# seemapoudel58/Physics_informed_image_segmentation

Hardware: AMD Instinct MI355X
Metric: training images/sec (512x512, Stage-II RD+PF loss) (higher is better)
Workload: dtype fp32 (fp16x3 split MFMA, power-of-two block scales; direct + Winograd convs); 1 GPU; C2: UNet(1,1,64) bs=8/GPU 512x512 Stage-II (lambda_RD=lambda_PF=1e-4, D=5, a=0.5, eps=0.05) AdamW lr=1e-5; global_batch=8, parallelism=dp1

## Files before the change

include/pis_capi.h:

```cpp
#ifndef PIS_CAPI_H
#define PIS_CAPI_H

#include <stddef.h>
#include <stdint.h>

#ifdef __cplusplus
extern "C" {
#endif

typedef void* pis_stream_t;

#define PIS_OK 0
#define PIS_ERR_ARG (-1)
#define PIS_ERR_LAUNCH (-2)
#define PIS_ERR_WORKSPACE (-3)

#define PIS_RELU 1
#define PIS_SCALE 2
#define PIS_MASK 4
#define PIS_ACCUMULATE 8
#define PIS_WINO_PREPARED 16
#define PIS_W_UNFLIPPED 32
#define PIS_FILTER_READY 64

// ... 27 lines not shown
#define PIS_TUNE_FUSED_STAGGER 25
#define PIS_TUNE_FUSED_WIDE 26
#define PIS_TUNE_FUSED_K128 27
#define PIS_TUNE_FUSED_PAIR 28
#define PIS_TUNE_DIRECT_H3 29
#define PIS_TUNE_DIRECT_WG 30
#define PIS_TUNE_WGRAD_T 31
#define PIS_TUNE_DIRECT_PIPE 32
#define PIS_TUNE_DIRECT_W8 33
#define PIS_TUNE_DIRECT_WSTRIP 34
#define PIS_TUNE_DIRECT_WBLOCKS 35
#define PIS_TUNE_HEAD_LOSS_ROWS 36
#define PIS_TUNE_DIRECT_WGRAD_ALL 37
#define PIS_TUNE_HEAD_LOSS_WIDE 38
#define PIS_TUNE_WGRAD_T_DEPTH 39
#define PIS_TUNE_DZ_VW 40
#define PIS_TUNE_GEMM_256 41
#define PIS_TUNE_LAST_WGRAD_MAIN 42
#define PIS_TUNE_DIRECT_W_VWALK 43
#define PIS_TUNE_DIRECT_WGRAD_MAIN 44
#define PIS_TUNE_GEMM_PRIO 45
#define PIS_TUNE_WINO_OUT_MPF 46
#define PIS_TUNE_WINO_F6 47
#define PIS_TUNE_WGRAD_OUT 48
#define PIS_TUNE_DIRECT_W_ROWS 49
#define PIS_TUNE_WINO_XFORM 50
#define PIS_TUNE_WINO_DGRAD_T 51
#define PIS_TUNE_PROB_VARIANT 52
#define PIS_TUNE_DIRECT_MFMA16 53
#define PIS_TUNE_EVOLVE_T 54
#define PIS_TUNE_EDT_PRUNE 55
#define PIS_TUNE_CONVT_WGRAD_TILE 56
#define PIS_TUNE_UNROLL_TB 57
#define PIS_TUNE_NKEYS 58
#define PIS_DEBUG_NOLOAD (1 << 16)
int pis_tune(int key, int value);
int pis_debug_gemm_nt(const float* A, const float* B, float* C, int M, int N, int K, int batch, int variant,
                      pis_stream_t stream);
int pis_debug_stream_probe(const float* a, const float* b, float* dst, int64_t n, float* partial, int grid,
                           pis_stream_t stream);

int pis_debug_band_probe(const float* a, int64_t n, int mode, float* partial, int grid, pis_stream_t stream);

int pis_arm_gemm_event(void* event);

int pis_stream_create(int priority, pis_stream_t* out);
int pis_stream_destroy(pis_stream_t stream);
int pis_stream_capture_status(pis_stream_t stream);

typedef void (*pis_launch_hook_t)(const char* kernel, int phase, pis_stream_t stream, double flop,
                                  void* user);
void pis_set_launch_hook(pis_launch_hook_t fn, void* user);

int pis_conv3x3_fwd(const float* x, int ldx, const float* w_krsc, const float* bias,
                    const float* scale, float* y, int ldy, int B, int H, int W, int Cin,
                    int Cout, int flags, pis_stream_t stream);
size_t pis_conv3x3_ex_ws(int B, int H, int W, int Cin, int Cout);
int pis_conv3x3_fwd_ex(const float* x, int ldx, const float* w_krsc, const float* bias,
                       const float* scale, float* y, int ldy, int B, int H, int W, int Cin, int Cout,
                       int flags, void* ws, size_t ws_bytes, pis_stream_t stream);
int pis_conv3x3_flip(const float* w_krsc, float* w_flip, int Cin, int Cout, pis_stream_t stream);
int pis_conv3x3_dgrad(const float* dz, int ldz, const float* w_flip, const float* mask, int ldm,
                      const float* scale, float* dx, int lddx, int B, int H, int W, int Cin,
                      int Cout, int flags, pis_stream_t stream);
int pis_conv3x3_dgrad_ex(const float* dz, int ldz, const float* w_flip, const float* mask, int ldm,
                         const float* scale, float* dx, int lddx, int B, int H, int W, int Cin,
                         int Cout, int flags, void* ws, size_t ws_bytes, pis_stream_t stream);
// ... 8 lines not shown
                           int B, int H, int W, int Cin, int Cout, int flags, void* ws, size_t ws_bytes,
                           const float* keep, pis_stream_t stream);
size_t pis_conv3x3_filter_bytes(int B, int H, int W, int Cin, int Cout, int dgrad);
int pis_conv3x3_filter(const float* w, int B, int H, int W, int Cin, int Cout, int dgrad, void* out,
                       size_t out_bytes, pis_stream_t stream);
typedef struct pis_filter_job {
  const float* w;
  void* out;
  size_t out_bytes;
  int B, H, W, Cin, Cout, dgrad;
} pis_filter_job;
#define PIS_FILTER_MAX_JOBS 40
int pis_conv3x3_filter_format(int B, int H, int W, int Cin, int Cout, int dgrad);
int pis_conv3x3_filters(const pis_filter_job* jobs, int n, pis_stream_t stream);
int pis_conv3x3_dgrad_direct(int B, int H, int W, int Cin, int Cout, int ldz, size_t ws_bytes);
int pis_conv3x3_bwd_prep(const float* dz, int ldz, int B, int H, int W, int Cin, int Cout, void* ws_dgrad,
                         size_t ws_dgrad_bytes, void* ws_wgrad, size_t ws_wgrad_bytes, pis_stream_t stream);
size_t pis_conv3x3_wgrad_ws(int B, int H, int W, int Cin, int Cout);
int pis_conv3x3_wgrad(const float* x, int ldx, const float* dz, int ldz, float* dw_krsc, float* db,
                      int B, int H, int W, int Cin, int Cout, int flags, void* ws, size_t ws_bytes,
                      pis_stream_t stream);

int pis_convt2x2_fwd(const float* x, int ldx, const float* w_ijoc, const float* bias, float* y,
                     int ldy, int B, int H, int W, int Cin, int Cout, pis_stream_t stream);
int pis_convt2x2_prep(const float* w_ijoc, float* w_cijo, int Cin, int Cout, pis_stream_t stream);
int pis_convt2x2_dgrad(const float* dy, int lddy, const float* w_cijo, const float* mask, int ldm,
                       float* dx, int lddx, int B, int H, int W, int Cin, int Cout, int flags,
                       pis_stream_t stream);
size_t pis_convt2x2_wgrad_ws(int B, int H, int W, int Cin, int Cout);
int pis_convt2x2_wgrad(const float* x, int ldx, const float* dy, int lddy, float* dw_ijoc,
                       float* db, int B, int H, int W, int Cin, int Cout, int flags, void* ws,
                       size_t ws_bytes, pis_stream_t stream);
int pis_debug_convt2x2_wgrad_tile_splits(int B, int H, int W, int Cin, int Cout);
int pis_debug_convt2x2_algo(int op, int B, int H, int W, int Cin, int Cout, int ld_src, int ld_dst, int aligned16);

int pis_maxpool2x2_fwd(const float* x, int ldx, float* y, int B, int H, int W, int C,
                       pis_stream_t stream);
int pis_maxpool2x2_bwd(const float* x, int ldx, const float* dy, const float* dskip, int ldskip,
                       float* dx, int lddx, int B, int H, int W, int C, pis_stream_t stream);

int pis_head_fwd(const float* x, int ldx, const float* w, const float* b, float* z, float* u,
                 int64_t npix, int C, pis_stream_t stream);
size_t pis_head_bwd_ws(int64_t npix, int C);
int pis_head_bwd(const float* x, int ldx, const float* w, const float* g, const float* u, float* dx,
                 int lddx, float* dw, float* db, int64_t npix, int C, int flags, void* ws,
                 size_t ws_bytes, pis_stream_t stream);

typedef struct pis_loss_params {
  float dice_w, bce_w;
  float rd_w, pf_w;
  float smooth;
  float D, a;
  float eps;
  float thr;
  int flags;
} pis_loss_params;
#define PIS_LOSS_ALL_TERMS 1
#define PIS_LOSS_CHAIN_SIGMOID 2
#define PIS_LOSS_NO_REACTION 4
#define PIS_LOSS_NTERMS 8
size_t pis_loss_ws(int B, int H, int W);
int pis_loss_fwd(const float* p, const float* t, int B, int H, int W, const pis_loss_params* prm,
                 float* out_terms, int* counts, float* scores, void* ws, size_t ws_bytes,
                 pis_stream_t stream);
int pis_loss_bwd(const float* p, const float* t, int B, int H, int W, const pis_loss_params* prm,
                 const float* terms, const float* grad_out, float* dst, int flags,
// ... 119 lines not shown
```

physics_informed_image_segmentation_amd/_hip.py:

```python
from __future__ import annotations

import ctypes
import os
from ctypes import c_double, c_float, c_int, c_int64, c_size_t, c_void_p
from typing import Optional

import torch

_HERE = os.path.dirname(os.path.abspath(__file__))
LIB_PATH = os.path.join(_HERE, "_lib", "libpis.so")

PIS_RELU, PIS_SCALE, PIS_MASK, PIS_ACCUMULATE, PIS_WINO_PREPARED, PIS_W_UNFLIPPED = 1, 2, 4, 8, 16, 32
PIS_FILTER_READY = 64
PIS_LOSS_ALL_TERMS, PIS_LOSS_CHAIN_SIGMOID, PIS_LOSS_NO_REACTION = 1, 2, 4
PIS_TUNE_LAST_WGRAD_MAIN = 42
PIS_TUNE_DIRECT_MFMA16 = 53
PIS_TUNE_PROB_VARIANT = 52
PIS_TUNE_EVOLVE_T = 54
PIS_TUNE_EDT_PRUNE = 55
PIS_TUNE_CONVT_WGRAD_TILE = 56
PIS_TUNE_UNROLL_TB = 57
PIS_UNROLL_MAX_STEPS = 1024
PIS_EVOLVE_CLAMP, PIS_EVOLVE_TILE_H, PIS_EVOLVE_TILE_W, PIS_EVOLVE_MAX_STEPS = 1, 32, 64, 65536
PIS_CACHE_IMG_U8, PIS_CACHE_IMG_F32, PIS_CACHE_MASK_BITS, PIS_CACHE_MASK_F32 = 0, 1, 0, 1
PIS_GRADNORM_SKIP_NONFINITE, PIS_GRADNORM_NSTATS = 1, 8
LOSS_NTERMS = 8
TERM_TOTAL, TERM_DICE, TERM_BCE, TERM_RD, TERM_PF, TERM_I, TERM_P, TERM_T = range(8)


class FilterJob(ctypes.Structure):
    _fields_ = [("w", c_void_p), ("out", c_void_p), ("out_bytes", c_size_t), ("B", c_int), ("H", c_int),
                ("W", c_int), ("Cin", c_int), ("Cout", c_int), ("dgrad", c_int)]


class LossParams(ctypes.Structure):
    _fields_ = [("dice_w", c_float), ("bce_w", c_float), ("rd_w", c_float), ("pf_w", c_float),
                ("smooth", c_float), ("D", c_float), ("a", c_float), ("eps", c_float),
                ("thr", c_float), ("flags", c_int)]


P, I, L, Z, Dbl = c_void_p, c_int, c_int64, c_size_t, c_double
LAUNCH_HOOK_T = ctypes.CFUNCTYPE(None, ctypes.c_char_p, c_int, c_void_p, ctypes.c_double, c_void_p)

_SIGNATURES = {
    "pis_set_launch_hook": ([LAUNCH_HOOK_T, P], None),
    "pis_arm_gemm_event": ([P], c_int),
    "pis_stream_create": ([I, ctypes.POINTER(c_void_p)], c_int),
    "pis_stream_destroy": ([P], c_int),
    "pis_stream_capture_status": ([P], c_int),
    "pis_version": ([], c_int),
    "pis_last_error": ([], ctypes.c_char_p),
    "pis_tune": ([I, I], c_int),
    "pis_debug_gemm_nt": ([P, P, P, I, I, I, I, I, P], c_int),
    "pis_debug_stream_probe": ([P, P, P, L, P, I, P], c_int),
    "pis_debug_band_probe": ([P, L, I, P, I, P], c_int),
    "pis_conv3x3_dgrad_direct": ([I, I, I, I, I, I, Z], c_int),
    "pis_conv3x3_bwd_prep": ([P, I, I, I, I, I, I, P, Z, P, Z, P], c_int),
    "pis_conv3x3_filter_bytes": ([I, I, I, I, I, I], c_size_t),
    "pis_conv3x3_filter_format": ([I, I, I, I, I, I], c_int),
    "pis_conv3x3_filter": ([P, I, I, I, I, I, I, P, Z, P], c_int),
    "pis_conv3x3_filters": ([P, I, P], c_int),
    "pis_conv3x3_fwd_pool": ([P, I, P, P, P, P, I, I, I, I, I, I, I, P, Z, P, P, P], c_int),
    "pis_conv3x3_fwd": ([P, I, P, P, P, P, I, I, I, I, I, I, I, P], c_int),
    "pis_conv3x3_flip": ([P, P, I, I, P], c_int),
    "pis_conv3x3_dgrad": ([P, I, P, P, I, P, P, I, I, I, I, I, I, I, P], c_int),
    "pis_conv3x3_ex_ws": ([I, I, I, I, I], c_size_t),
    "pis_conv3x3_fwd_ex": ([P, I, P, P, P, P, I, I, I, I, I, I, I, P, Z, P], c_int),
    "pis_conv3x3_dgrad_ex": ([P, I, P, P, I, P, P, I, I, I, I, I, I, I, P, Z, P], c_int),
    "pis_conv3x3_wgrad_ws": ([I, I, I, I, I], c_size_t),
    "pis_conv3x3_keep_bytes": ([I, I, I, I, I], c_size_t),
    "pis_conv3x3_fwd_keep": ([P, I, P, P, P, P, I, I, I, I, I, I, I, P, Z, P, P], c_int),
    "pis_conv3x3_wgrad_keep": ([P, I, P, I, P, P, I, I, I, I, I, I, P, Z, P, P], c_int),
    "pis_conv3x3_wgrad": ([P, I, P, I, P, P, I, I, I, I, I, I, P, Z, P], c_int),
    "pis_convt2x2_fwd": ([P, I, P, P, P, I, I, I, I, I, I, P], c_int),
    "pis_convt2x2_prep": ([P, P, I, I, P], c_int),
    "pis_convt2x2_dgrad": ([P, I, P, P, I, P, I, I, I, I, I, I, I, P], c_int),
    "pis_convt2x2_wgrad_ws": ([I, I, I, I, I], c_size_t),
    "pis_convt2x2_wgrad": ([P, I, P, I, P, P, I, I, I, I, I, I, P, Z, P], c_int),
    "pis_debug_convt2x2_wgrad_tile_splits": ([I, I, I, I, I], c_int),
    "pis_debug_convt2x2_algo": ([I, I, I, I, I, I, I, I, I], c_int),
    "pis_maxpool2x2_fwd": ([P, I, P, I, I, I, I, P], c_int),
    "pis_maxpool2x2_bwd": ([P, I, P, P, I, P, I, I, I, I, I, P], c_int),
    "pis_head_fwd": ([P, I, P, P, P, P, L, I, P], c_int),
    "pis_head_bwd_ws": ([L, I], c_size_t),
    "pis_head_bwd": ([P, I, P, P, P, P, I, P, P, L, I, I, P, Z, P], c_int),
    "pis_loss_ws": ([I, I, I], c_size_t),
    "pis_loss_fwd": ([P, P, I, I, I, ctypes.POINTER(LossParams), P, P, P, P, Z, P], c_int),
    "pis_loss_bwd": ([P, P, I, I, I, ctypes.POINTER(LossParams), P, P, P, I, P], c_int),
    "pis_head_loss_fwd_ws": ([I, I, I], c_size_t),
    "pis_head_loss_fwd_ok": ([I, I, I, I], c_int),
    "pis_head_loss_fwd": ([P, I, P, P, P, P, P, I, I, I, I, ctypes.POINTER(LossParams), P, P, P, P, Z, P], c_int),
    "pis_head_loss_bwd_ws": ([I, I, I, I], c_size_t),
    "pis_head_loss_bwd": ([P, I, P, P, P, P, I, I, I, I, ctypes.POINTER(LossParams), P, P, P, I, P, P, I, P, Z,
                           P], c_int),
    "pis_adamw_step": ([P, P, P, P, L, Dbl, Dbl, Dbl, Dbl, Dbl, Dbl, Dbl, Dbl, P], c_int),
    "pis_grad_sumsq_ws": ([I, L], c_size_t),
    "pis_grad_sumsq": ([P, P, P, I, Dbl, Dbl, I, P, P, P, P, Z, P], c_int),
    "pis_adamw_step_clipped": ([P, P, P, P, L, Dbl, Dbl, Dbl, Dbl, Dbl, Dbl, Dbl, Dbl, P, P], c_int),
    "pis_adamw_step_ema": ([P, P, P, P, P, L, Dbl, Dbl, Dbl, Dbl, Dbl, Dbl, Dbl, Dbl, Dbl, P, P], c_int),
    "pis_arena_exchange": ([P, P, L, P], c_int),
    "pis_colsum_ws": ([L, I], c_size_t),
    "pis_colsum": ([P, I, L, I, P, I, P, Z, P], c_int),
    "pis_pde_fields": ([P, I, I, I, c_float, c_float, P, P, P, P], c_int),
    "pis_pde_fields_bwd": ([P, P, P, P, I, I, I, c_float, c_float, P, P], c_int),
    "pis_synth_ws": ([I, I, I], c_size_t),
    "pis_synth_discs": ([P, P, I, ctypes.c_uint64, P, P, P, I, I, I, P, Z, P], c_int),
    "pis_boundary_ws": ([I, I, I], c_size_t),
    "pis_boundary_metrics": ([P, P, I, I, I, c_float, I, P, P, P, P, Z, P], c_int),
    "pis_objects_ws": ([I, I, I], c_size_t),
    "pis_object_metrics": ([P, P, I, I, I, c_float, I, I, P, P, P, P, Z, P], c_int),
    "pis_probability_ws": ([I, I, I], c_size_t),
    "pis_probability_table": ([P, P, I, I, I, P, P, P, Z, P], c_int),
    "pis_cache_batch": ([P, I, Z, P, I, Z, P, P, P, L, P, P, I, I, I, P], c_int),
# ... 163 lines not shown
```

physics_informed_image_segmentation_amd/csrc/capi.hip:

```cpp
#include <atomic>
#include <cstdarg>

#include "common.h"

namespace pis {
static thread_local char g_last_error[512] = "";

void set_error(const char* fmt, ...) {
  va_list ap;
  va_start(ap, fmt);
  vsnprintf(g_last_error, sizeof(g_last_error), fmt, ap);
  va_end(ap);
}

static std::atomic<int> g_tune[PIS_TUNE_NKEYS] = {0, 16, 0, 1, 0, 1, 512, 0, 1, 1024, 4, 1, 0, 4, 3, 1, 1, 2,
                                                   1, 1, 1, 0, 1, 0, 0, 0, 2, 1, 0, 1, 0, 1, 1, 0, 0, 512, 0, 0, 1, 2, 2, 0, 1, 1, 0, 0, 1,
                                                   0, 1, 2, 1, 1, 0, 3, 8, 3, 1, 2};

int tune_get(int key) { return (key > 0 && key < PIS_TUNE_NKEYS) ? g_tune[key].load() : 0; }

static std::atomic<pis_launch_hook_t> g_hook{nullptr};
static std::atomic<void*> g_hook_user{nullptr};

void launch_hook(const char* kernel, int phase, hipStream_t s, double flop) {
  const pis_launch_hook_t fn = g_hook.load(std::memory_order_relaxed);
  if (fn) fn(kernel, phase, (pis_stream_t)s, flop, g_hook_user.load(std::memory_order_relaxed));
}

static thread_local hipEvent_t g_gemm_event = nullptr;

void gemm_done(hipStream_t s) {
  if (g_gemm_event) {
    (void)hipEventRecord(g_gemm_event, s);
    g_gemm_event = nullptr;
  }
}
}

extern "C" const char* pis_last_error(void) { return pis::g_last_error; }
extern "C" int pis_version(void) { return 1; }

extern "C" int pis_arm_gemm_event(void* event) {
  const int pending = pis::g_gemm_event != nullptr;
  pis::g_gemm_event = (hipEvent_t)event;
  return pending;
}

extern "C" int pis_stream_create(int priority, pis_stream_t* out) {
  PIS_CHECK_ARG(out != nullptr, "pis_stream_create: out is NULL");
  hipStream_t s = nullptr;
// ... 60 lines not shown
```

physics_informed_image_segmentation_amd/csrc/conv3x3_plan.h:

```cpp
#pragma once
#include "igemm.h"

namespace pis {

struct WgradPlan {
  int bm, bn, splits, pps;
  size_t part_bytes, bias_bytes;
};
WgradPlan plan_wgrad(int Mp, int Np, int P, int group_m, int group_n, int target_blocks = 2048);
size_t wgrad_ws_bytes(const WgradPlan& pl);
size_t colsum_ws(int64_t npix, int C);

enum class WgradKernel {
  F32,
  X6,
  H3_COLS,
  H3T,
  H3T_EXACT,
  H3T_TWIN,
};
constexpr int WT_BK = 32;
struct WgradOperands {
  bool plain;
  bool a_up2;
  int W, P, Np;
  int lda, ldb;
  int64_t bs_a, bs_b;
  bool aligned16;
};
bool h3t_exact(const WgradPlan& pl, const WgradOperands& o);
WgradKernel choose_wgrad_kernel(const WgradPlan& pl, const WgradOperands& o);

struct HaloPlan {
  bool use;
  int splits, seg_per_split, nseg;
  size_t part_bytes, bias_bytes;
};

struct WinoWgradPlan {
  bool use, fused_bias, gemm_bias;
  int m, nxi;
  int64_t T;
  WgradPlan gemm;
  size_t off_E, off_part, off_M, off_cs, total;
};

constexpr int C1_BLOCKS = 1024;

enum WgradAlgo {
  WGRAD_NONE = 0,
  WGRAD_DIRECT,
  WGRAD_WINO4,
  WGRAD_WINO2,
  WGRAD_HALO,
  WGRAD_C1_STREAM,
  WGRAD_C1_MFMA,
  WGRAD_GENERIC,
};

enum PrepKind {
  PREP_NONE = 0,
  PREP_DZ2,
  PREP_DZ2_TMAX,
  PREP_E_ONLY,
};

struct ConvDirPlan {
  int C, N;
  bool direct;
  bool wino_wanted;
  ConvAlgo wino;
  ConvAlgo wino_kept;
  ConvAlgo fallback;
  size_t direct_ws, wino_ws;
  int filter_format;
  size_t filter_bytes;
// ... 37 lines not shown
```

physics_informed_image_segmentation_amd/csrc/conv3x3_plan.hip:

```cpp
#include "conv3x3_plan.h"

namespace pis {
namespace {

int wino_tile(int H, int W) { return (tune_get(PIS_TUNE_WINO_F4) != 0 && H % 4 == 0 && W % 4 == 0) ? 4 : 2; }

bool direct_h3_wanted(int H, int W, int C, int N) {
  const int mode = tune_get(PIS_TUNE_DIRECT_H3);
  if (mode == 0 || !direct_h3_shape_ok(H, W, C, N, 4)) return false;
  const int lo = std::min(C, N), hi = std::max(C, N);
  if (mode == 3)
    return (H >= 256 && hi <= 256) || (H >= 128 && hi <= 256 && lo <= 128);
  if (mode == 4)
    return H >= 128 && hi <= 256;
  if (mode == 5)
    return H >= 128;
  return mode == 2 || (hi <= 128 && H >= 256);
}

bool wino_wanted_dims(int H, int W, int C, int N) {
  const int mode = tune_get(PIS_TUNE_WINOGRAD);
  if (mode == 0 || H % 2 || W % 2 || C % 4 || N % 4) return false;
  if (mode == 2) return true;
  if (wino_tile(H, W) == 4)
// ... 8 lines not shown
         T >= 2 * (int64_t)C &&
         (C == 64 || (C == 128 && tune_get(PIS_TUNE_FUSED_K128) != 0)) &&
         (N == 64 || (N % 64 == 0 && N <= 64 * (1 << tune_get(PIS_TUNE_FUSED_WIDE))));
}

bool wino6_layer(int B, int H, int W, int Cin, int Cout) {
  if (tune_get(PIS_TUNE_WINO_F6) == 0 || tune_get(PIS_TUNE_WINO_TILE) != 4 || B <= 0) return false;
  if (wino_tile(H, W) != 4 || Cin % 64 || Cout % 64) return false;
  if (direct_h3_wanted(H, W, Cin, Cout) || direct_h3_wanted(H, W, Cout, Cin)) return false;
  if (!wino_wanted_dims(H, W, Cin, Cout) || !wino_wanted_dims(H, W, Cout, Cin)) return false;
  if (wino_fused_wanted(B, H, W, Cin, Cout) || wino_fused_wanted(B, H, W, Cout, Cin)) return false;
  const int64_t p6 = (int64_t)64 * ((H + 5) / 6) * ((W + 5) / 6), p4 = (int64_t)36 * (H / 4) * (W / 4);
  return 10 * p6 <= 9 * p4;
}

HaloPlan halo_plan(int B, int H, int W, int Cin, int Cout) {
  HaloPlan p{};
  p.use = Cin % 64 == 0 && Cout % 64 == 0 && W % 16 == 0;
  if (!p.use) return p;
  p.nseg = (int)((int64_t)B * H * W / 16);
  const int tiles = (Cout / 64) * (Cin / 64);
  const size_t slab = (size_t)Cout * 9 * Cin * sizeof(float);
  int64_t splits = cdiv(std::max(64, tune_get(PIS_TUNE_WGRAD_BLOCKS)), tiles);
  splits = std::min<int64_t>(splits, std::max<int64_t>(1, (int64_t)((160u << 20) / slab)));
  int64_t sps = cdiv(p.nseg, splits);
  sps = std::max<int64_t>(32, std::min<int64_t>(512, sps));
  p.seg_per_split = (int)sps;
  p.splits = (int)cdiv(p.nseg, sps);
  p.part_bytes = (size_t)p.splits * slab;
  p.bias_bytes = (size_t)p.splits * Cout * sizeof(float);
  return p;
}

WinoWgradPlan wino_wgrad_plan(int B, int H, int W, int Cin, int Cout) {
  WinoWgradPlan p{};
  const int mode = tune_get(PIS_TUNE_WINOGRAD);
  const int m = wino_tile(H, W);
  const bool wanted = m == 4 || (Cin >= 128 && Cout >= 128);
  p.use = mode != 0 && H % 2 == 0 && W % 2 == 0 && Cin % 64 == 0 && Cout % 64 == 0 && (mode == 2 || wanted);
  if (!p.use) return p;
  p.m = m;
  p.nxi = (p.m + 2) * (p.m + 2);
  p.T = (int64_t)B * (H / p.m) * (W / p.m);
  p.gemm = plan_wgrad(Cout, Cin, (int)p.T, Cout, Cin, std::max(16, tune_get(PIS_TUNE_WINO_WGRAD_BLOCKS) / p.nxi));
  auto al = [](size_t b) { return cdiv(b, 256) * 256; };
  const size_t V = al((size_t)p.nxi * p.T * Cin * 4), E = al((size_t)p.nxi * p.T * Cout * 4);
  const size_t part = al((size_t)p.gemm.splits * p.nxi * Cout * Cin * 4), M = al((size_t)p.nxi * Cout * Cin * 4);
  p.off_E = V;
  p.off_part = V + E;
  p.off_M = p.off_part + part;
  p.off_cs = p.off_M + M;
  p.gemm_bias = p.m == 4 && ((int64_t)Cout * Cin) % 64 == 0;
  p.fused_bias = false;
  const size_t cs = p.gemm_bias ? (size_t)p.gemm.splits * Cout * sizeof(float) : colsum_ws((int64_t)B * H * W, Cout);
  p.total = p.off_cs + al(cs) + 256;
  return p;
}

int filter_format(const Conv3x3Plan& p, const ConvDirPlan& d, bool is_dgrad, bool wino6) {
  if (p.B <= 0 || p.H <= 0 || p.W <= 0 || p.Cin % 4 || p.Cout % 4 || p.Cin < 4) return 0;
  if (wino6) return 4;
  if (d.direct) return 3;
  if (is_dgrad ? (p.Cin % 32 || p.Cout % 32 || !d.wino_wanted) : (p.keep_bytes == 0 && !d.wino_wanted)) return 0;
  return d.wino_kept == ALGO_WINO4_FUSED ? 2 : wino_tile(p.H, p.W) == 4 ? 1 : 0;
}

size_t filter_bytes(const Conv3x3Plan& p, const ConvDirPlan& d) {
  const size_t nc = (size_t)36 * p.Cin * p.Cout;
  switch (d.filter_format) {
    case 1: return nc * sizeof(float);
    case 2:
      return p.fused_h3 ? 2 * nc * sizeof(_Float16) + (size_t)d.N * sizeof(float) : 3 * nc * sizeof(__bf16);
    case 3: return d.direct_ws;
    case 4: return (size_t)64 * p.Cin * p.Cout * sizeof(float);
    default: return 0;
  }
}

ConvDirPlan plan_dir(int B, int H, int W, int C, int N, bool is_dgrad, bool wino6) {
  ConvDirPlan d{};
  d.C = C;
  d.N = N;
  d.direct = direct_h3_wanted(H, W, C, N);
  d.direct_ws = direct_h3_ws_bytes(C, N);
  d.wino_wanted = wino_wanted_dims(H, W, C, N);
  const int m = wino_tile(H, W);
  if (H % 2 || W % 2 || C % 4 || N % 4) d.wino_kept = ALGO_NONE;
  else if (m != 4) d.wino_kept = ALGO_WINO2;
  else if (wino_fused_wanted(B, H, W, C, N)) d.wino_kept = ALGO_WINO4_FUSED;
  else if (is_dgrad && tune_get(PIS_TUNE_WINO_DGRAD_T) != 0) d.wino_kept = ALGO_WINO4_DGRAD_T;
  else d.wino_kept = ALGO_WINO4_GEMM;
  d.wino = (wino6 && d.wino_kept != ALGO_NONE) ? ALGO_WINO6 : d.wino_kept;
  d.wino_ws = wino_ws_bytes(m, B, H, W, C, N);
  if (wino6) d.wino_ws = std::max(d.wino_ws, wino6_ws_bytes(B, H, W, C, N));
  if (!is_dgrad && C == 1) d.fallback = (N == 64 && W % 64 == 0) ? ALGO_C1_ROW : ALGO_C1_STREAM;
  else d.fallback = (tune_get(PIS_TUNE_CONV_HALO) && W % 16 == 0 && H % 8 == 0 && C % 4 == 0) ? ALGO_HALO : ALGO_IGEMM;
  return d;
}

}

bool h3t_exact(const WgradPlan& pl, const WgradOperands& o) {
  return o.P % WT_BK == 0 && pl.pps % WT_BK == 0 &&
         ((int64_t)o.P + WT_BK) * std::max(o.a_up2 ? 0 : o.lda, o.ldb) * 4 < (int64_t(1) << 31);
}

WgradKernel choose_wgrad_kernel(const WgradPlan& pl, const WgradOperands& o) {
  const int x6 = tune_get(PIS_TUNE_WGRAD_X6);
  const bool cols = o.plain && pl.pps % 16 == 0 && (!o.a_up2 || o.W % 8 == 0);
  if (cols && (x6 == 2 || (x6 == 3 && o.Np >= 256))) {
    if (tune_get(PIS_TUNE_WGRAD_T) != 0 && pl.bm == 128 && pl.bn == 128 && !o.a_up2 && pl.pps % WT_BK == 0 &&
        o.lda % 4 == 0 && o.ldb % 4 == 0 && o.bs_a % 4 == 0 && o.bs_b % 4 == 0 && o.aligned16)
      return tune_get(PIS_TUNE_DEBUG_NOLOAD) ? WgradKernel::H3T_TWIN
             : h3t_exact(pl, o)              ? WgradKernel::H3T_EXACT
                                             : WgradKernel::H3T;
    return WgradKernel::H3_COLS;
  }
  return (cols && x6 != 0) ? WgradKernel::X6 : WgradKernel::F32;
}

Conv3x3Plan plan_conv3x3(int B, int H, int W, int Cin, int Cout) {
  Conv3x3Plan p{};
  p.B = B; p.H = H; p.W = W; p.Cin = Cin; p.Cout = Cout;
  const bool wino6 = wino6_layer(B, H, W, Cin, Cout);
  p.fwd = plan_dir(B, H, W, Cin, Cout, false, wino6);
  p.dgrad = plan_dir(B, H, W, Cout, Cin, true, wino6);
  p.fused_h3 = tune_get(PIS_TUNE_WINO_GEMM_OUT_H3) != 0;

  const bool direct_w = direct_w_shape_ok(B, H, W, Cin, Cout, 4, 4) && p.fwd.direct;
  p.wino_w = wino_wgrad_plan(B, H, W, Cin, Cout);
  p.halo_w = halo_plan(B, H, W, Cin, Cout);
  if (Cout % 64 == 0 && (Cin == 1 || Cin % 64 == 0)) {
    if (p.wino_w.use) {
      p.wgrad_nodirect = p.wino_w.m == 4 ? WGRAD_WINO4 : WGRAD_WINO2;
      p.wgrad_ws_nodirect = p.wino_w.total;
    } else if (p.halo_w.use) {
      p.wgrad_nodirect = WGRAD_HALO;
      p.wgrad_ws_nodirect = cdiv(p.halo_w.part_bytes, 256) * 256 + p.halo_w.bias_bytes + 256;
    } else if (Cin == 1 && tune_get(PIS_TUNE_C1_WGRAD) == 0) {
      p.wgrad_nodirect = WGRAD_C1_STREAM;
// ... 35 lines not shown
  const auto fail = [](const char* msg) { return set_error("%s", msg), ALGO_NONE; };
  const bool strides_ok = c.lds % 4 == 0 && c.ldd % 4 == 0 && (!c.masked || c.ldm % 4 == 0);
  const bool direct_ok = c.has_ws && d.direct && c.lds % 4 == 0;
  if (c.w_unflipped && !c.prepared && !(direct_ok && c.ws_bytes >= d.direct_ws) &&
      !(c.has_ws && d.wino == ALGO_WINO6 && strides_ok && c.ws_bytes >= d.wino_ws))
    return fail("pis_conv3x3_dgrad_ex: PIS_W_UNFLIPPED needs the prepared F(4x4,3x3) path, the F(6x6,3x3) one or the "
                "direct one");
  if (direct_ok && !c.prepared && (c.filter_ready || c.ws_bytes >= d.direct_ws)) return ALGO_DIRECT_H3;
  const ConvAlgo w = (c.kept || c.prepared) ? d.wino_kept : d.wino;
  if (c.has_ws && w != ALGO_NONE && strides_ok && (c.kept || d.wino_wanted) && c.ws_bytes >= d.wino_ws) {
    if (c.filter_ready && w == ALGO_WINO2) return fail("launch_wino3x3: PIS_FILTER_READY needs the F(4x4,3x3) GEMM path");
    if (w == ALGO_WINO2 && c.prepared) return fail("launch_wino3x3: prepared transforms need F(4x4,3x3)");
    if (w != ALGO_WINO6 && w != ALGO_WINO4_FUSED && c.w_unflipped && (w == ALGO_WINO2 || d.N % 32 || d.C % 32))
      return fail("launch_wino3x3: unflipped weights need F(4x4,3x3) and 32-aligned channels");
    return w;
  }
  if (c.filter_ready) return fail("conv3x3: PIS_FILTER_READY but this call does not take the F(4x4,3x3) path");
  if (c.prepared)
    return fail("pis_conv3x3_dgrad_ex: PIS_WINO_PREPARED but this call does not take the Winograd path");
  return (d.fallback == ALGO_HALO && c.lds % 4 != 0) ? ALGO_IGEMM : d.fallback;
}

WgradAlgo resolve_wgrad(const Conv3x3Plan& p, const void* x, const void* dz, size_t ws_bytes) {
  if (p.wgrad != WGRAD_DIRECT) return p.wgrad_nodirect;
  if (((uintptr_t)x & 15) == 0 && ((uintptr_t)dz & 15) == 0 && ws_bytes >= p.wgrad_ws) return WGRAD_DIRECT;
  if (ws_bytes >= p.wgrad_ws_nodirect) return p.wgrad_nodirect;
  set_error("pis_conv3x3_wgrad: x / dz not 16-byte aligned or workspace below the direct kernel's; "
            "the non-direct fallback needs a larger "
            "workspace than pis_conv3x3_wgrad_ws reports for this (direct) layer");
  return WGRAD_NONE;
}

}
```

physics_informed_image_segmentation_amd/csrc/wgrad.hip:

```cpp
#include "convt_plan.h"

namespace pis {

enum BMode { B_PLAIN = 0, B_CONV3 = 1, B_CONV3_C1 = 2 };

struct WgradArgs {
  const float* a; int lda; int a_up2; int Ca;
  const float* b; int ldb; int b_mode; int Cb;
  int B, H, W;
  int P;
  int Mp, Np;
  int pix_per_split;
  float* part;
  float* part_bias;
  int64_t bs_a, bs_b, bs_part, split_stride;
  int pair;
  int bias_xi;
  int dbg;
};

template <int BM, int BN, int BKP>
__global__ __launch_bounds__(256) void wgrad_f32_kernel(WgradArgs g) {
  const Remap2 rm = xcd_remap2();
  if (rm.batch) {
// ... 1274 lines not shown
    if (more) {
      split_store((st + 1) & 1);
      if (st + 2 < nst) gload(st + 2);
    }
  }
  float* out = g.part + (size_t)split * g.Mp * g.Np;
  const float inv_a = ua != 0.f ? 1.f / ua : 0.f, inv_b = ub != 0.f ? 1.f / ub : 0.f;
#pragma unroll
  for (int a = 0; a < 4; ++a)
#pragma unroll
    for (int b = 0; b < 2; ++b) {
      const int n = n0 + 64 * wn + 32 * b + li;
#pragma unroll
      for (int r = 0; r < 16; ++r) {
        const int m = m0 + 128 * wm + 32 * a + (r & 3) + 8 * (r >> 2) + 4 * lh;
        out[(size_t)m * g.Np + n] = (acc[a][b][r] * inv_a) * inv_b;
      }
    }
  if (do_bias) {
    f32x4* rb4 = reinterpret_cast<f32x4*>(smem);
    rb4[tid] = bsum[0];
    rb4[256 + tid] = bsum[1];
    __syncthreads();
    if (tid < 64) {
      const int base = 256 * (tid >> 5) + (tid & 31);
      f32x4 t = rb4[base];
#pragma unroll
      for (int r = 1; r < 8; ++r) t += rb4[base + 32 * r];
      *reinterpret_cast<f32x4*>(g.part_bias + (size_t)split * g.Mp + m0 + 4 * tid) = t;
    }
  }
}

static WgradOperands wgrad_operands(const WgradArgs& a) {
  return {a.b_mode == B_PLAIN, a.a_up2 != 0, a.W, a.P, a.Np, a.lda, a.ldb, a.bs_a, a.bs_b,
          (((uintptr_t)a.a | (uintptr_t)a.b) & 15) == 0};
}

static int run_wgrad(const WgradArgs& base, const WgradPlan& pl, WgradKernel k, hipStream_t s, int batches = 1) {
  WgradArgs a = base;
  a.pix_per_split = pl.pps;
  a.pair = tune_get(PIS_TUNE_WGRAD_PAIR);
  a.dbg = tune_get(PIS_TUNE_DEBUG_NOLOAD);
  const int tiles = (a.Mp / pl.bm) * (a.Np / pl.bn);
  const dim3 grid(tiles * pl.splits, batches);
  using Kernel = void (*)(WgradArgs);
  static const Kernel f32[4] = {wgrad_f32_kernel<64, 64, 32>, wgrad_f32_kernel<64, 128, 32>, wgrad_f32_kernel<128, 64, 32>,
                                wgrad_f32_kernel<128, 128, 16>};
  static const Kernel x6[4] = {wgrad_x6_kernel<64, 64>, wgrad_x6_kernel<64, 128>, wgrad_x6_kernel<128, 64>,
                               wgrad_x6_kernel<128, 128>};
  static const Kernel h3[4] = {wgrad_h3_kernel<64, 64>, wgrad_h3_kernel<64, 128>, wgrad_h3_kernel<128, 64>,
                               wgrad_h3_kernel<128, 128>};
  const int t = (pl.bm == 128 ? 2 : 0) + (pl.bn == 128 ? 1 : 0);
  const bool up2 = a.a_up2 != 0;
  Kernel fn = f32[t];
  const char* name = "wgrad_f32";
  switch (k) {
    case WgradKernel::F32: break;
    case WgradKernel::X6: fn = x6[t]; name = "wgrad_x6"; break;
    case WgradKernel::H3_COLS: fn = h3[t]; name = "wgrad_h3"; break;
    case WgradKernel::H3T: fn = up2 ? wgrad_h3t_kernel<true, 2> : wgrad_h3t_kernel<false, 2>; break;
    case WgradKernel::H3T_EXACT: fn = up2 ? wgrad_h3t_kernel<true, 2, false, true> : wgrad_h3t_kernel<false, 2, false, true>; break;
    case WgradKernel::H3T_TWIN: fn = wgrad_h3t_kernel<false, 2, true>; break;
  }
  if (k >= WgradKernel::H3T) name = up2 ? "wgrad_h3t<up2>" : "wgrad_h3t";
  hipLaunchKernelGGL(fn, grid, dim3(256), 0, s, a);
  return launch_status(name);
}

}

using namespace pis;

extern "C" size_t pis_colsum_ws(int64_t npix, int C) { return colsum_ws(npix, C); }

extern "C" int pis_colsum(const float* src, int ld, int64_t npix, int C, float* out, int flags,
                          void* ws, size_t ws_bytes, pis_stream_t stream) {
  PIS_CHECK_ARG(src && out && npix > 0 && C > 0, "pis_colsum: bad arguments");
  PIS_CHECK_ARG(C % 4 != 0 || ld % 4 == 0, "pis_colsum: ld must be a multiple of 4");
  PIS_CHECK_ARG(ld >= C, "pis_colsum: ld must be at least C");
  PIS_CHECK_ARG(ws && ws_bytes >= colsum_ws(npix, C), "pis_colsum: workspace missing or too small");
  PIS_CHECK_ARG(C % 4 != 0 || ((uintptr_t)src | (uintptr_t)ws) % 16 == 0,
                "pis_colsum: src and ws must be 16-byte aligned when C is a multiple of 4");
  return colsum(src, ld, npix, C, out, flags & PIS_ACCUMULATE, ws, ws_bytes, (hipStream_t)stream);
}

__global__ __launch_bounds__(256) void wgrad_c1_kernel(const float* __restrict__ x, int ldx,
                                                       const float* __restrict__ dz, int ldz, int B, int H,
                                                       int W, int Cout, int64_t pix_per_block,
                                                       float* __restrict__ part, float* __restrict__ part_b) {
  __shared__ f32x4 red[256][10];
  const int lanes = Cout / 4, groups = 256 / lanes;
  const int lp = threadIdx.x / lanes, q = threadIdx.x - lp * lanes, c4 = 4 * q;
  f32x4 acc[10];
#pragma unroll
  for (int k = 0; k < 10; ++k) acc[k] = f32x4{0.f, 0.f, 0.f, 0.f};
  const int HW = H * W;
  const int64_t npix = (int64_t)B * HW;
// ... 74 lines not shown
  __syncthreads();
  for (int o = tid; o < 10 * Cout; o += 256) {
    const int n = o / 10, k = o - n * 10, qq = n >> 2, j = n & 3;
    float sum = 0.f;
    for (int gi = 0; gi < 16; ++gi) sum += red[gi * 16 + qq][k][j];
    if (k < 9) part[(size_t)blockIdx.x * 9 * Cout + n * 9 + k] = sum;
    else if (part_b) part_b[(size_t)blockIdx.x * Cout + n] = sum;
  }
}

static int wino_wgrad(const float* x, int ldx, const float* dz, int ldz, float* dw, float* db, int B, int H, int W,
                      int Cin, int Cout, int acc, const WinoWgradPlan& p, void* ws, hipStream_t s,
                      const float* keep_v = nullptr, bool e_ready = false) {
  char* base = (char*)ws;
  float* V = (float*)base;
  float* E = (float*)(base + p.off_E);
  float* part = (float*)(base + p.off_part);
  float* M = (float*)(base + p.off_M);
  int rc = 0;
  if (keep_v && p.m == 4) V = const_cast<float*>(keep_v);
  else rc = launch_wino_input(x, ldx, B, H, W, Cin, V, s, p.m);
  if (!rc && !e_ready) rc = launch_wino_dz(dz, ldz, B, H, W, Cout, E, s, p.m, nullptr);
  if (rc) return rc;
  float* gbias = (db && p.gemm_bias) ? (float*)(base + p.off_cs) : nullptr;
  WgradArgs a{};
  a.a = E; a.lda = Cout; a.a_up2 = 0; a.Ca = Cout;
  a.b = V; a.ldb = Cin; a.b_mode = B_PLAIN; a.Cb = Cin;
  a.B = 1; a.H = 1; a.W = (int)p.T; a.P = (int)p.T; a.Mp = Cout; a.Np = Cin;
  a.part = part; a.part_bias = gbias; a.bias_xi = WINO4_BIAS_XI;
  a.bs_a = p.T * Cout; a.bs_b = p.T * Cin; a.bs_part = (int64_t)Cout * Cin;
  a.split_stride = (int64_t)p.nxi * Cout * Cin;
  const double flop = 2.0 * p.nxi * (double)p.T * Cout * Cin;
  launch_hook("wino_wgrad_gemm", 0, s, flop);
  rc = run_wgrad(a, p.gemm, choose_wgrad_kernel(p.gemm, wgrad_operands(a)), s, p.nxi);
  launch_hook("wino_wgrad_gemm", 1, s, flop);
  const WgradOutBias bf{gbias, gbias ? p.gemm.splits : 0, db, WINO4_BIAS_SCALE};
  if (p.m == 4 && p.gemm.splits <= 16) {
    if (!rc) rc = launch_wino_wgrad_out(part, Cout, Cin, dw, acc, s, p.m, p.gemm.splits, a.split_stride, bf);
  } else {
    if (!rc) rc = reduce_slabs_pitched(part, p.gemm.splits, a.split_stride, a.split_stride, M, 0, s);
    if (!rc) rc = launch_wino_wgrad_out(M, Cout, Cin, dw, acc, s, p.m, 1, 0, bf);
  }
  if (!rc && db && !gbias) rc = colsum(dz, ldz, (int64_t)B * H * W, Cout, db, acc, base + p.off_cs, p.total - p.off_cs, s);
  return rc;
}

__global__ void compact_c1_kernel(const float* __restrict__ full, float* __restrict__ dw, int Cout,
                                  int accumulate) {
  const int i = blockIdx.x * blockDim.x + threadIdx.x;
  if (i >= Cout * 9) return;
  const int n = i / 9, t = i - n * 9;
  const float v = full[n * 64 + t];
  dw[i] = accumulate ? dw[i] + v : v;
}

extern "C" size_t pis_conv3x3_wgrad_ws(int B, int H, int W, int Cin, int Cout) {
  return plan_conv3x3(B, H, W, Cin, Cout).wgrad_ws;
}

extern "C" int pis_conv3x3_wgrad_keep(const float* x, int ldx, const float* dz, int ldz, float* dw_krsc,
                                      float* db, int B, int H, int W, int Cin, int Cout, int flags, void* ws,
                                      size_t ws_bytes, const float* keep, pis_stream_t stream) {
  const Conv3x3Plan p = plan_conv3x3(B, H, W, Cin, Cout);
  const WinoWgradPlan& wp = p.wino_w;
  const bool prepared = flags & PIS_WINO_PREPARED;
  PIS_CHECK_ARG(!prepared || (keep && wp.use && wp.m == 4),
                "pis_conv3x3_wgrad_keep: PIS_WINO_PREPARED needs the kept-transform F(3x3,4x4) path");
  const bool direct = p.wgrad == WGRAD_DIRECT && ldx % 4 == 0 && ldz % 4 == 0;
  if (!keep || !(wp.use && wp.m == 4) || (!prepared && direct))
    return pis_conv3x3_wgrad(x, ldx, dz, ldz, dw_krsc, db, B, H, W, Cin, Cout, flags, ws, ws_bytes, stream);
  PIS_CHECK_ARG(x && dz && dw_krsc && ldz % 4 == 0, "pis_conv3x3_wgrad_keep: bad arguments");
  PIS_CHECK_ARG(ws && ws_bytes >= wp.total, "pis_conv3x3_wgrad_keep: workspace too small");
  return wino_wgrad(x, ldx, dz, ldz, dw_krsc, db, B, H, W, Cin, Cout, flags & PIS_ACCUMULATE, wp, ws,
// ... 144 lines not shown
```

Baseline: 394.5 images/s.

## Add larger-tile Winograd wgrad GEMM kernel with occupancy-trimmed split plan

Measured after the change: 399.4 images/s (median of 6 runs). 1.01x the previous value.

```diff
diff --git a/include/pis_capi.h b/include/pis_capi.h
--- a/include/pis_capi.h
+++ b/include/pis_capi.h
@@ -83,7 +83,8 @@
 #define PIS_TUNE_EDT_PRUNE 55
 #define PIS_TUNE_CONVT_WGRAD_TILE 56
 #define PIS_TUNE_UNROLL_TB 57
-#define PIS_TUNE_NKEYS 58
+#define PIS_TUNE_WINO_WGRAD_TILE 58
+#define PIS_TUNE_NKEYS 59
 #define PIS_DEBUG_NOLOAD (1 << 16)
 int pis_tune(int key, int value);
 int pis_debug_gemm_nt(const float* A, const float* B, float* C, int M, int N, int K, int batch, int variant,
@@ -158,6 +159,8 @@
                        float* db, int B, int H, int W, int Cin, int Cout, int flags, void* ws,
                        size_t ws_bytes, pis_stream_t stream);
 int pis_debug_convt2x2_wgrad_tile_splits(int B, int H, int W, int Cin, int Cout);
+int pis_debug_wino_wgrad_kernel(int B, int H, int W, int Cin, int Cout, int aligned);
+int pis_debug_wino_wgrad_plan(int B, int H, int W, int Cin, int Cout, int aligned, int* splits, int* blocks);
 int pis_debug_convt2x2_algo(int op, int B, int H, int W, int Cin, int Cout, int ld_src, int ld_dst, int aligned16);
 
 int pis_maxpool2x2_fwd(const float* x, int ldx, float* y, int B, int H, int W, int C,
diff --git a/physics_informed_image_segmentation_amd/_hip.py b/physics_informed_image_segmentation_amd/_hip.py
--- a/physics_informed_image_segmentation_amd/_hip.py
+++ b/physics_informed_image_segmentation_amd/_hip.py
@@ -20,6 +20,7 @@
 PIS_TUNE_EDT_PRUNE = 55
 PIS_TUNE_CONVT_WGRAD_TILE = 56
 PIS_TUNE_UNROLL_TB = 57
+PIS_TUNE_WINO_WGRAD_TILE = 58
 PIS_UNROLL_MAX_STEPS = 1024
 PIS_EVOLVE_CLAMP, PIS_EVOLVE_TILE_H, PIS_EVOLVE_TILE_W, PIS_EVOLVE_MAX_STEPS = 1, 32, 64, 65536
 PIS_CACHE_IMG_U8, PIS_CACHE_IMG_F32, PIS_CACHE_MASK_BITS, PIS_CACHE_MASK_F32 = 0, 1, 0, 1
@@ -79,6 +80,8 @@
     "pis_convt2x2_wgrad": ([P, I, P, I, P, P, I, I, I, I, I, I, P, Z, P], c_int),
     "pis_debug_convt2x2_wgrad_tile_splits": ([I, I, I, I, I], c_int),
     "pis_debug_convt2x2_algo": ([I, I, I, I, I, I, I, I, I], c_int),
+    "pis_debug_wino_wgrad_kernel": ([I, I, I, I, I, I], c_int),
+    "pis_debug_wino_wgrad_plan": ([I, I, I, I, I, I, ctypes.POINTER(c_int), ctypes.POINTER(c_int)], c_int),
     "pis_maxpool2x2_fwd": ([P, I, P, I, I, I, I, P], c_int),
     "pis_maxpool2x2_bwd": ([P, I, P, P, I, P, I, I, I, I, I, P], c_int),
     "pis_head_fwd": ([P, I, P, P, P, P, L, I, P], c_int),
diff --git a/physics_informed_image_segmentation_amd/csrc/capi.hip b/physics_informed_image_segmentation_amd/csrc/capi.hip
--- a/physics_informed_image_segmentation_amd/csrc/capi.hip
+++ b/physics_informed_image_segmentation_amd/csrc/capi.hip
@@ -15,7 +15,7 @@
 
 static std::atomic<int> g_tune[PIS_TUNE_NKEYS] = {0, 16, 0, 1, 0, 1, 512, 0, 1, 1024, 4, 1, 0, 4, 3, 1, 1, 2,
                                                    1, 1, 1, 0, 1, 0, 0, 0, 2, 1, 0, 1, 0, 1, 1, 0, 0, 512, 0, 0, 1, 2, 2, 0, 1, 1, 0, 0, 1,
-                                                   0, 1, 2, 1, 1, 0, 3, 8, 3, 1, 2};
+                                                   0, 1, 2, 1, 1, 0, 3, 8, 3, 1, 2, 1};
 
 int tune_get(int key) { return (key > 0 && key < PIS_TUNE_NKEYS) ? g_tune[key].load() : 0; }
 
diff --git a/physics_informed_image_segmentation_amd/csrc/conv3x3_plan.h b/physics_informed_image_segmentation_amd/csrc/conv3x3_plan.h
--- a/physics_informed_image_segmentation_amd/csrc/conv3x3_plan.h
+++ b/physics_informed_image_segmentation_amd/csrc/conv3x3_plan.h
@@ -18,6 +18,7 @@
   H3T,
   H3T_EXACT,
   H3T_TWIN,
+  H3T_TILE,
 };
 constexpr int WT_BK = 32;
 struct WgradOperands {
@@ -29,7 +30,7 @@
   bool aligned16;
 };
 bool h3t_exact(const WgradPlan& pl, const WgradOperands& o);
-WgradKernel choose_wgrad_kernel(const WgradPlan& pl, const WgradOperands& o);
+WgradKernel choose_wgrad_kernel(const WgradPlan& pl, const WgradOperands& o, const WgradPlan* tile = nullptr);
 
 struct HaloPlan {
   bool use;
@@ -42,6 +43,7 @@
   int m, nxi;
   int64_t T;
   WgradPlan gemm;
+  WgradPlan tile;
   size_t off_E, off_part, off_M, off_cs, total;
 };
 
diff --git a/physics_informed_image_segmentation_amd/csrc/conv3x3_plan.hip b/physics_informed_image_segmentation_amd/csrc/conv3x3_plan.hip
--- a/physics_informed_image_segmentation_amd/csrc/conv3x3_plan.hip
+++ b/physics_informed_image_segmentation_amd/csrc/conv3x3_plan.hip
@@ -64,6 +64,35 @@
   return p;
 }
 
+constexpr int WINO_TILE_RESIDENT = 512;
+
+bool wino_tile_adopted(int Cin, int Cout, bool trimmed) {
+  return std::min(Cin, Cout) == 128 || trimmed || (Cin == Cout && Cin >= 512);
+}
+
+WgradPlan wino_tile_plan(const WinoWgradPlan& p, int Cin, int Cout) {
+  WgradPlan t{};
+  const int key = tune_get(PIS_TUNE_WINO_WGRAD_TILE);
+  if (key == 0 || p.T % WT_BK || p.T < 512 || Cin % 128 || Cout % 128 || (Cin % 256 && Cout % 256)) return t;
+  const bool trim = key != 2;
+  bool trimmed = false;
+  t = p.gemm;
+  t.bm = Cout % 256 == 0 ? 256 : 128;
+  t.bn = Cout % 256 == 0 ? 128 : 256;
+  const int tiles = (Cout / t.bm) * (Cin / t.bn);
+  const int fit = WINO_TILE_RESIDENT / (tiles * p.nxi);
+  if (trim && t.splits > 1 && tiles * t.splits * p.nxi > WINO_TILE_RESIDENT && fit >= 2) {
+    const int64_t pps = cdiv(cdiv(p.T, (int64_t)fit), WT_BK) * WT_BK;
+    if (pps <= 8192) {
+      t.pps = (int)pps;
+      t.splits = (int)cdiv(p.T, pps);
+      trimmed = true;
+    }
+  }
+  if (key == 1 && !wino_tile_adopted(Cin, Cout, trimmed)) return WgradPlan{};
+  return t;
+}
+
 WinoWgradPlan wino_wgrad_plan(int B, int H, int W, int Cin, int Cout) {
   WinoWgradPlan p{};
   const int mode = tune_get(PIS_TUNE_WINOGRAD);
@@ -75,6 +104,7 @@
   p.nxi = (p.m + 2) * (p.m + 2);
   p.T = (int64_t)B * (H / p.m) * (W / p.m);
   p.gemm = plan_wgrad(Cout, Cin, (int)p.T, Cout, Cin, std::max(16, tune_get(PIS_TUNE_WINO_WGRAD_BLOCKS) / p.nxi));
+  p.tile = wino_tile_plan(p, Cin, Cout);
   auto al = [](size_t b) { return cdiv(b, 256) * 256; };
   const size_t V = al((size_t)p.nxi * p.T * Cin * 4), E = al((size_t)p.nxi * p.T * Cout * 4);
   const size_t part = al((size_t)p.gemm.splits * p.nxi * Cout * Cin * 4), M = al((size_t)p.nxi * Cout * Cin * 4);
@@ -137,7 +167,11 @@
          ((int64_t)o.P + WT_BK) * std::max(o.a_up2 ? 0 : o.lda, o.ldb) * 4 < (int64_t(1) << 31);
 }
 
-WgradKernel choose_wgrad_kernel(const WgradPlan& pl, const WgradOperands& o) {
+WgradKernel choose_wgrad_kernel(const WgradPlan& pl, const WgradOperands& o, const WgradPlan* tile) {
+  if (tile && tile->bm != 0 && o.plain && !o.a_up2 && tune_get(PIS_TUNE_WGRAD_X6) >= 2 && tune_get(PIS_TUNE_WGRAD_T) != 0 &&
+      tune_get(PIS_TUNE_DEBUG_NOLOAD) == 0 && o.lda % 4 == 0 && o.ldb % 4 == 0 && o.bs_a % 4 == 0 && o.bs_b % 4 == 0 &&
+      o.aligned16 && h3t_exact(*tile, o))
+    return WgradKernel::H3T_TILE;
   const int x6 = tune_get(PIS_TUNE_WGRAD_X6);
   const bool cols = o.plain && pl.pps % 16 == 0 && (!o.a_up2 || o.W % 8 == 0);
   if (cols && (x6 == 2 || (x6 == 3 && o.Np >= 256))) {
@@ -239,3 +273,25 @@
 }
 
 }
+
+using namespace pis;
+
+extern "C" int pis_debug_wino_wgrad_plan(int B, int H, int W, int Cin, int Cout, int aligned, int* splits, int* blocks) {
+  if (splits) *splits = 0;
+  if (blocks) *blocks = 0;
+  if (B <= 0 || H <= 0 || W <= 0 || Cin <= 0 || Cout <= 0) return -1;
+  const Conv3x3Plan p = plan_conv3x3(B, H, W, Cin, Cout);
+  const WgradAlgo algo = (p.wgrad == WGRAD_DIRECT && aligned) ? WGRAD_DIRECT : p.wgrad_nodirect;
+  if (algo != WGRAD_WINO4 && algo != WGRAD_WINO2) return -1;
+  const WinoWgradPlan& w = p.wino_w;
+  const WgradOperands o{true, false, (int)w.T, (int)w.T, Cin, Cout, Cin, w.T * Cout, w.T * Cin, aligned != 0};
+  const WgradKernel k = choose_wgrad_kernel(w.gemm, o, &w.tile);
+  const WgradPlan& pl = k == WgradKernel::H3T_TILE ? w.tile : w.gemm;
+  if (splits) *splits = pl.splits;
+  if (blocks) *blocks = (Cout / pl.bm) * (Cin / pl.bn) * pl.splits * w.nxi;
+  return (int)k | (k == WgradKernel::H3T_TILE ? (pl.bm == 256 ? 1 : 2) << 4 : 0);
+}
+
+extern "C" int pis_debug_wino_wgrad_kernel(int B, int H, int W, int Cin, int Cout, int aligned) {
+  return pis_debug_wino_wgrad_plan(B, H, W, Cin, Cout, aligned, nullptr, nullptr);
+}
diff --git a/physics_informed_image_segmentation_amd/csrc/wgrad.hip b/physics_informed_image_segmentation_amd/csrc/wgrad.hip
--- a/physics_informed_image_segmentation_amd/csrc/wgrad.hip
+++ b/physics_informed_image_segmentation_amd/csrc/wgrad.hip
@@ -1330,6 +1330,201 @@
   }
 }
 
+template <bool WB>
+__global__ __launch_bounds__(256, 2) void wgrad_h3t_tile_kernel(WgradArgs g) {
+  const Remap2 rm = xcd_remap2();
+  if (rm.batch) {
+    g.a += rm.batch * g.bs_a;
+    g.b += rm.batch * g.bs_b;
+    g.part += rm.batch * g.bs_part;
+  }
+  constexpr int BMT = WB ? 128 : 256, BNT = WB ? 256 : 128;
+  constexpr int HA = WB ? 1 : 2, HB = WB ? 2 : 1;
+  constexpr int NA = WB ? 2 : 4, NB = WB ? 4 : 2;
+  __shared__ __attribute__((aligned(16))) _Float16 smem[WU_LDS];
+  __shared__ float red[2][2][4];
+  const int tid = threadIdx.x, lane = tid & 63, wave = tid >> 6;
+  const int w0 = wave & 1, w1 = wave >> 1, li = lane & 31, lh = lane >> 5;
+  const int ntn = g.Np / BNT;
+  const int tiles = (g.Mp / BMT) * ntn;
+  const int bid = rm.bid;
+  const int split = bid / tiles;
+  const int tile = bid - split * tiles;
+  const int m0 = (tile / ntn) * BMT, n0 = (tile % ntn) * BNT;
+  const int p_begin = split * g.pix_per_split;
+  const int p_end = min(g.P, p_begin + g.pix_per_split);
+  const int nst = max(0, (p_end - p_begin) / WT_BK);
+  const int srow = tid >> 5, sc4 = tid & 31;
+  const bool do_bias = g.part_bias != nullptr && n0 == 0 && rm.batch == g.bias_xi;
+  f32x4 bsum[HA];
+#pragma unroll
+  for (int h = 0; h < HA; ++h) bsum[h] = f32x4{0.f, 0.f, 0.f, 0.f};
+
+  const __amdgpu_buffer_rsrc_t rsa = __builtin_amdgcn_make_buffer_rsrc(const_cast<float*>(g.a + m0), (short)0, 0x7fffffff, 0x00020000);
+  const __amdgpu_buffer_rsrc_t rsb = __builtin_amdgcn_make_buffer_rsrc(const_cast<float*>(g.b + n0), (short)0, 0x7fffffff, 0x00020000);
+  const uint32_t la0 = 4u * ((uint32_t)(p_begin + srow) * (uint32_t)g.lda + 4u * sc4);
+  const uint32_t lb0 = 4u * ((uint32_t)(p_begin + srow) * (uint32_t)g.ldb + 4u * sc4);
+  f32x4 xa[HA][4], xb[HB][4];
+  auto gload = [&](int st) __attribute__((always_inline)) {
+    const uint32_t ra_s = 4u * (uint32_t)(st * WT_BK) * (uint32_t)g.lda, rb_s = 4u * (uint32_t)(st * WT_BK) * (uint32_t)g.ldb;
+#pragma unroll
+    for (int j = 0; j < 4; ++j) {
+#pragma unroll
+      for (int h = 0; h < HA; ++h)
+        xa[h][j] = __builtin_bit_cast(f32x4, __builtin_amdgcn_raw_buffer_load_b128(rsa, la0, ra_s + 4u * (uint32_t)(8 * j) * (uint32_t)g.lda + 512u * h, 0));
+#pragma unroll
+      for (int h = 0; h < HB; ++h)
+        xb[h][j] = __builtin_bit_cast(f32x4, __builtin_amdgcn_raw_buffer_load_b128(rsb, lb0, rb_s + 4u * (uint32_t)(8 * j) * (uint32_t)g.ldb + 512u * h, 0));
+    }
+  };
+  auto publish = [&](int par) __attribute__((always_inline)) {
+    if (do_bias) {
+#pragma unroll
+      for (int j = 0; j < 4; ++j)
+#pragma unroll
+        for (int h = 0; h < HA; ++h) bsum[h] += xa[h][j];
+    }
+    const float ma = wave_max_nonneg(absmax_x4(xa));
+    const float mb = wave_max_nonneg(absmax_x4(xb));
+    if (lane == 0) {
+      red[par][0][wave] = ma;
+      red[par][1][wave] = mb;
+    }
+  };
+  float sa = 0.f, sb = 0.f, sa_min = __builtin_inff(), sb_min = __builtin_inff();
+  auto split_store = [&](int par) __attribute__((always_inline)) {
+    sa = h3_keep(sa, umax4(red[par][0]), sa_min);
+    sb = h3_keep(sb, umax4(red[par][1]), sb_min);
+#pragma unroll
+    for (int j = 0; j < 4; ++j) {
+      const int off = wtsw(srow + 8 * j, sc4 >> 1) + 4 * (sc4 & 1);
+      u32x2 h, l;
+#pragma unroll
+      for (int hf = 0; hf < HA; ++hf) {
+        split2h_x4(xa[hf][j] * sa, h, l);
+        *reinterpret_cast<u32x2*>(smem + hf * WT_PLANE + off) = h;
+        *reinterpret_cast<u32x2*>(smem + (HA + hf) * WT_PLANE + off) = l;
+      }
+#pragma unroll
+      for (int hf = 0; hf < HB; ++hf) {
+        split2h_x4(xb[hf][j] * sb, h, l);
+        *reinterpret_cast<u32x2*>(smem + (2 * HA + hf) * WT_PLANE + off) = h;
+        *reinterpret_cast<u32x2*>(smem + (2 * HA + HB + hf) * WT_PLANE + off) = l;
+      }
+    }
+  };
+
+  const int gq = lane >> 4, q = (lane & 15) >> 2, pp = lane & 3;
+  const int kh = gq >> 1, chk = 2 * (gq & 1) + (pp >> 1), slot = 4 * (pp & 1);
+  auto frag = [&](const _Float16* plane, int ks, int col0) __attribute__((always_inline)) {
+    const int row = 16 * ks + 8 * kh + q, ch = col0 / 8 + chk;
+    const s16x4 lo4 = tr_read(plane + wtsw(row, ch) + slot);
+    const s16x4 hi4 = tr_read(plane + wtsw(row + 4, ch) + slot);
+    return __builtin_bit_cast(f16x8, __builtin_shufflevector(lo4, hi4, 0, 1, 2, 3, 4, 5, 6, 7));
+  };
+  const _Float16* a_hi = smem + (WB ? 0 : w0) * WT_PLANE;
+  const _Float16* a_lo = a_hi + HA * WT_PLANE;
+  const _Float16* b_hi = smem + (2 * HA + (WB ? w0 : 0)) * WT_PLANE;
+  const _Float16* b_lo = b_hi + HB * WT_PLANE;
+  const int ca0 = WB ? 64 * w1 : 0, cb0 = WB ? 0 : 64 * w1;
+
+  f32x16 acc[NA][NB];
+#pragma unroll
+  for (int a = 0; a < NA; ++a)
+#pragma unroll
+    for (int b = 0; b < NB; ++b)
+#pragma unroll
+      for (int r = 0; r < 16; ++r) acc[a][b][r] = 0.f;
+  float ua = 0.f, ub = 0.f;
+
+  if (nst > 0) {
+    gload(0);
+    publish(0);
+    __syncthreads();
+    split_store(0);
+    if (nst > 1) gload(1);
+  }
+#pragma unroll 1
+  for (int st = 0; st < nst; ++st) {
+    __syncthreads();
+    if (sa != ua || sb != ub) {
+      if (ua != 0.f) {
+        const float fa = sa / ua, fb = sb / ub;
+#pragma unroll
+        for (int a = 0; a < NA; ++a)
+#pragma unroll
+          for (int b = 0; b < NB; ++b) acc[a][b] = (acc[a][b] * fa) * fb;
+      }
+      ua = sa;
+      ub = sb;
+    }
+#pragma unroll
+    for (int ks = 0; ks < 2; ++ks) {
+      if constexpr (!WB) {
+        f16x8 bf[2][NB];
+#pragma unroll
+        for (int b = 0; b < NB; ++b) {
+          bf[0][b] = frag(b_hi, ks, cb0 + 32 * b);
+          bf[1][b] = frag(b_lo, ks, cb0 + 32 * b);
+        }
+#pragma unroll
+        for (int a = 0; a < NA; ++a) {
+          const f16x8 ah = frag(a_hi, ks, ca0 + 32 * a), al = frag(a_lo, ks, ca0 + 32 * a);
+#pragma unroll
+          for (int b = 0; b < NB; ++b) acc[a][b] = h3_mfma3(ah, al, bf[0][b], bf[1][b], acc[a][b]);
+        }
+      } else {
+        f16x8 af[2][NA];
+#pragma unroll
+        for (int a = 0; a < NA; ++a) {
+          af[0][a] = frag(a_hi, ks, ca0 + 32 * a);
+          af[1][a] = frag(a_lo, ks, ca0 + 32 * a);
+        }
+#pragma unroll
+        for (int b = 0; b < NB; ++b) {
+          const f16x8 bh = frag(b_hi, ks, cb0 + 32 * b), bl = frag(b_lo, ks, cb0 + 32 * b);
+#pragma unroll
+          for (int a = 0; a < NA; ++a) acc[a][b] = h3_mfma3(af[0][a], af[1][a], bh, bl, acc[a][b]);
+        }
+      }
+    }
+    const bool more = st + 1 < nst;
+    if (more) publish((st + 1) & 1);
+    __syncthreads();
+    if (more) {
+      split_store((st + 1) & 1);
+      if (st + 2 < nst) gload(st + 2);
+    }
+  }
+  float* out = g.part + (size_t)split * (g.split_stride ? g.split_stride : (int64_t)g.Mp * g.Np);
+  const float inv_a = ua != 0.f ? 1.f / ua : 0.f, inv_b = ub != 0.f ? 1.f / ub : 0.f;
+  const int mw = m0 + (WB ? 64 * w1 : 128 * w0), nw = n0 + (WB ? 128 * w0 : 64 * w1);
+#pragma unroll
+  for (int a = 0; a < NA; ++a)
+#pragma unroll
+    for (int b = 0; b < NB; ++b) {
+      const int n = nw + 32 * b + li;
+#pragma unroll
+      for (int r = 0; r < 16; ++r) {
+        const int m = mw + 32 * a + (r & 3) + 8 * (r >> 2) + 4 * lh;
+        out[(size_t)m * g.Np + n] = (acc[a][b][r] * inv_a) * inv_b;
+      }
+    }
+  if (do_bias) {
+    f32x4* rb4 = reinterpret_cast<f32x4*>(smem);
+#pragma unroll
+    for (int h = 0; h < HA; ++h) rb4[256 * h + tid] = bsum[h];
+    __syncthreads();
+    if (tid < 32 * HA) {
+      const int base = 256 * (tid >> 5) + (tid & 31);
+      f32x4 t = rb4[base];
+#pragma unroll
+      for (int r = 1; r < 8; ++r) t += rb4[base + 32 * r];
+      *reinterpret_cast<f32x4*>(g.part_bias + (size_t)split * g.Mp + m0 + 4 * tid) = t;
+    }
+  }
+}
+
 static WgradOperands wgrad_operands(const WgradArgs& a) {
   return {a.b_mode == B_PLAIN, a.a_up2 != 0, a.W, a.P, a.Np, a.lda, a.ldb, a.bs_a, a.bs_b,
           (((uintptr_t)a.a | (uintptr_t)a.b) & 15) == 0};
@@ -1360,8 +1555,9 @@
     case WgradKernel::H3T: fn = up2 ? wgrad_h3t_kernel<true, 2> : wgrad_h3t_kernel<false, 2>; break;
     case WgradKernel::H3T_EXACT: fn = up2 ? wgrad_h3t_kernel<true, 2, false, true> : wgrad_h3t_kernel<false, 2, false, true>; break;
     case WgradKernel::H3T_TWIN: fn = wgrad_h3t_kernel<false, 2, true>; break;
-  }
-  if (k >= WgradKernel::H3T) name = up2 ? "wgrad_h3t<up2>" : "wgrad_h3t";
+    case WgradKernel::H3T_TILE: fn = pl.bn == 256 ? wgrad_h3t_tile_kernel<true> : wgrad_h3t_tile_kernel<false>; break;
+  }
+  if (k >= WgradKernel::H3T) name = k == WgradKernel::H3T_TILE ? "wgrad_h3t_tile" : up2 ? "wgrad_h3t<up2>" : "wgrad_h3t";
   hipLaunchKernelGGL(fn, grid, dim3(256), 0, s, a);
   return launch_status(name);
 }
@@ -1502,13 +1698,15 @@
   a.split_stride = (int64_t)p.nxi * Cout * Cin;
   const double flop = 2.0 * p.nxi * (double)p.T * Cout * Cin;
   launch_hook("wino_wgrad_gemm", 0, s, flop);
-  rc = run_wgrad(a, p.gemm, choose_wgrad_kernel(p.gemm, wgrad_operands(a)), s, p.nxi);
+  const WgradKernel kern = choose_wgrad_kernel(p.gemm, wgrad_operands(a), &p.tile);
+  const WgradPlan& gp = kern == WgradKernel::H3T_TILE ? p.tile : p.gemm;
+  rc = run_wgrad(a, gp, kern, s, p.nxi);
   launch_hook("wino_wgrad_gemm", 1, s, flop);
-  const WgradOutBias bf{gbias, gbias ? p.gemm.splits : 0, db, WINO4_BIAS_SCALE};
-  if (p.m == 4 && p.gemm.splits <= 16) {
-    if (!rc) rc = launch_wino_wgrad_out(part, Cout, Cin, dw, acc, s, p.m, p.gemm.splits, a.split_stride, bf);
+  const WgradOutBias bf{gbias, gbias ? gp.splits : 0, db, WINO4_BIAS_SCALE};
+  if (p.m == 4 && gp.splits <= 16) {
+    if (!rc) rc = launch_wino_wgrad_out(part, Cout, Cin, dw, acc, s, p.m, gp.splits, a.split_stride, bf);
   } else {
-    if (!rc) rc = reduce_slabs_pitched(part, p.gemm.splits, a.split_stride, a.split_stride, M, 0, s);
+    if (!rc) rc = reduce_slabs_pitched(part, gp.splits, a.split_stride, a.split_stride, M, 0, s);
     if (!rc) rc = launch_wino_wgrad_out(M, Cout, Cin, dw, acc, s, p.m, 1, 0, bf);
   }
   if (!rc && db && !gbias) rc = colsum(dz, ldz, (int64_t)B * H * W, Cout, db, acc, base + p.off_cs, p.total - p.off_cs, s);
```
